# dongzhuoyao/self-guided-diffusion-models

Hardware: AMD Instinct MI355X
Metric: cfg_sampled_images_per_sec_64x64_1000step_ddpm (higher is better)
Workload: dtype f32 as 3xf16 split MFMA products, f32 accumulate; 1 GPU; IN64 unet_fast ch128 cluster-k5000 cond_scale=2 bs=40/GPU (UNet batch 80), 1000-step native DDPM; batch_per_gpu=40, unet_batch=80, precision_mode=f16x3, launch=hipGraph-captured step

## Files before the change

self-guided-diffusion-models_amd/csrc/attention.hip:

```cpp
#include "sgdm_common.h"
#include "../../include/sgdm_hip.h"

namespace {

constexpr int KT = 64;

template <int D>
__global__ __launch_bounds__(256) void attention_kernel(const float* __restrict__ q, int q_ld, int q_hs,
                                                        const float* __restrict__ k, const float* __restrict__ v,
                                                        int kv_ld, int kv_hs, int tq, int tk, float scale,
                                                        float* __restrict__ out, int out_ld,
                                                        float* __restrict__ lse,
                                                        const uint8_t* __restrict__ kmask = nullptr) {
    constexpr int LD = D + 4;
    constexpr int DT = (D + 31) / 32;
    constexpr int KT = D > 64 ? 32 : 64;
    __shared__ __attribute__((aligned(16))) float Ks[KT * LD];
    __shared__ __attribute__((aligned(16))) float Vs[KT * LD];

    const int tid = threadIdx.x, lane = tid & 63, wave = tid >> 6;
    const int li = lane & 31, lh = lane >> 5;
    const int head = blockIdx.y, b = blockIdx.z;
    const int qi = blockIdx.x * 128 + wave * 32 + li;
    const int qc = qi < tq ? qi : tq - 1;

    f32x4 qreg[D / 8];
    {
        const float* qp = q + ((long)b * tq + qc) * q_ld + head * q_hs;
#pragma unroll
        for (int s = 0; s < D / 8; ++s) {
            f32x4 t = *reinterpret_cast<const f32x4*>(qp + s * 8 + lh * 4);
            qreg[s] = t * scale;
        }
    }

    f32x16 oacc[DT];
#pragma unroll
    for (int i = 0; i < DT; ++i)
#pragma unroll
        for (int r = 0; r < 16; ++r) oacc[i][r] = 0.f;
    float m_run = -INFINITY, l_run = 0.f;

    const float* kb = k + (long)b * tk * kv_ld + head * kv_hs;
    const float* vb = v + (long)b * tk * kv_ld + head * kv_hs;

    for (int kt0 = 0; kt0 < tk; kt0 += KT) {
        __syncthreads();
        constexpr int VPR = D / 4;
        for (int idx = tid; idx < KT * VPR; idx += 256) {
            const int row = idx / VPR, c4 = idx % VPR;
            f32x4 kv4 = {0.f, 0.f, 0.f, 0.f}, vv4 = {0.f, 0.f, 0.f, 0.f};
            if (kt0 + row < tk) {
                kv4 = *reinterpret_cast<const f32x4*>(kb + (long)(kt0 + row) * kv_ld + c4 * 4);
                vv4 = *reinterpret_cast<const f32x4*>(vb + (long)(kt0 + row) * kv_ld + c4 * 4);
            }
            *reinterpret_cast<f32x4*>(Ks + row * LD + c4 * 4) = kv4;
            *reinterpret_cast<f32x4*>(Vs + row * LD + c4 * 4) = vv4;
        }
        __syncthreads();

#pragma unroll
        for (int st = 0; st < KT / 32; ++st) {
            if (kt0 + st * 32 >= tk) break;
            f32x16 sacc;
#pragma unroll
            for (int r = 0; r < 16; ++r) sacc[r] = 0.f;
#pragma unroll
            for (int s = 0; s < D / 8; ++s) {
                f32x4 kf = *reinterpret_cast<const f32x4*>(Ks + (st * 32 + li) * LD + s * 8 + lh * 4);
#pragma unroll
                for (int j = 0; j < 4; ++j) sacc = __builtin_amdgcn_mfma_f32_32x32x2f32(kf[j], qreg[s][j], sacc, 0, 0, 0);
            }
            unsigned dead = 0;
            if (kmask) {
#pragma unroll
                for (int r = 0; r < 16; ++r) {
                    const int key = kt0 + st * 32 + (r & 3) + 8 * (r >> 2) + 4 * lh;
                    const uint8_t keep = kmask[(long)b * tk + (key < tk ? key : tk - 1)];
                    dead |= (keep ? 0u : 1u) << r;
                }
            }
            float mx = -INFINITY;
#pragma unroll
            for (int r = 0; r < 16; ++r) {
                const int key = kt0 + st * 32 + (r & 3) + 8 * (r >> 2) + 4 * lh;
                const bool drop = key >= tk || ((dead >> r) & 1u);
                sacc[r] = drop ? -INFINITY : sacc[r];
                mx = fmaxf(mx, sacc[r]);
            }
            mx = fmaxf(mx, __shfl_xor(mx, 32, 64));
            const float m_new = fmaxf(m_run, mx);
            const float alpha = __expf(m_run - m_new);
            float psum = 0.f;
#pragma unroll
            for (int r = 0; r < 16; ++r) {
                sacc[r] = __expf(sacc[r] - m_new);
                psum += sacc[r];
            }
            l_run = l_run * alpha + psum;
            m_run = m_new;
#pragma unroll
            for (int dt = 0; dt < DT; ++dt) {
#pragma unroll
                for (int r = 0; r < 16; ++r) oacc[dt][r] *= alpha;
#pragma unroll
                for (int r = 0; r < 16; ++r) {
                    const int key = st * 32 + (r & 3) + 8 * (r >> 2) + 4 * lh;
                    float vf = 0.f;
                    if (D >= 32 || li < D) vf = Vs[key * LD + dt * 32 + li];
                    oacc[dt] = __builtin_amdgcn_mfma_f32_32x32x2f32(vf, sacc[r], oacc[dt], 0, 0, 0);
                }
            }
        }
    }
    const float l_tot = l_run + __shfl_xor(l_run, 32, 64);
    const float inv = 1.0f / l_tot;
    if (lse && qi < tq && lh == 0) lse[((long)b * gridDim.y + head) * tq + qi] = m_run + __logf(l_tot);
    if (qi < tq) {
        float* op = out + ((long)b * tq + qi) * out_ld + head * D;
#pragma unroll
        for (int dt = 0; dt < DT; ++dt)
#pragma unroll
            for (int r = 0; r < 16; ++r) {
                const int dd = dt * 32 + (r & 3) + 8 * (r >> 2) + 4 * lh;
                if (dd < D) op[dd] = oacc[dt][r] * inv;
            }
    }
}


__device__ __forceinline__ void split_f16(float v, _Float16& hi, _Float16& lo) {
    SGD_ROUNDED(v);
    hi = (_Float16)v;
    lo = (_Float16)(v - (float)hi);
}

template <int D>
__global__ __launch_bounds__(256) void attention_split_kernel(const float* __restrict__ q, int q_ld, int q_hs,
                                                              const float* __restrict__ k, const float* __restrict__ v,
                                                              int kv_ld, int kv_hs, int tq, int tk, float scale,
                                                              float* __restrict__ out, int out_ld,
                                                              float* __restrict__ lse) {
    constexpr int DT = (D + 31) / 32;
    constexpr int DP = DT * 32;
    constexpr int KS = (D + 15) / 16;
    constexpr int DK = KS * 16;
    constexpr int KT = D > 64 ? 32 : 64;
    constexpr int LDK = DK + 8;
    constexpr int LDV = KT + 8;
    __shared__ __attribute__((aligned(16))) _Float16 Kh[KT * LDK];
    __shared__ __attribute__((aligned(16))) _Float16 Kl[KT * LDK];
    __shared__ __attribute__((aligned(16))) _Float16 Vh[DP * LDV];
    __shared__ __attribute__((aligned(16))) _Float16 Vl[DP * LDV];

    const int tid = threadIdx.x, lane = tid & 63, wave = tid >> 6;
    const int li = lane & 31, lh = lane >> 5;
    const int head = blockIdx.y, b = blockIdx.z;
    const int qi = blockIdx.x * 128 + wave * 32 + li;
    const int qc = qi < tq ? qi : tq - 1;

    f16x8 qh[KS], ql[KS];
    {
        const float* qp = q + ((long)b * tq + qc) * q_ld + head * q_hs;
#pragma unroll
        for (int s = 0; s < KS; ++s)
#pragma unroll
            for (int j4 = 0; j4 < 2; ++j4) {
                const int c = s * 16 + lh * 8 + j4 * 4;
                f32x4 t = {0.f, 0.f, 0.f, 0.f};
                if (c < D) t = *reinterpret_cast<const f32x4*>(qp + c);
#pragma unroll
                for (int j = 0; j < 4; ++j) {
                    _Float16 h, l;
                    split_f16(t[j] * scale, h, l);
                    qh[s][j4 * 4 + j] = h;
                    ql[s][j4 * 4 + j] = l;
                }
            }
    }

    f32x16 oacc[DT];
#pragma unroll
    for (int i = 0; i < DT; ++i)
#pragma unroll
        for (int r = 0; r < 16; ++r) oacc[i][r] = 0.f;
    float m_run = -INFINITY, l_run = 0.f;
    constexpr float LOG2E = 1.4426950408889634f;
    constexpr float PSHIFT = 14.0f;

    const float* kb = k + (long)b * tk * kv_ld + head * kv_hs;
    const float* vb = v + (long)b * tk * kv_ld + head * kv_hs;

    if (DP > D) {
        for (int idx = tid; idx < (DP - D) * LDV; idx += 256) {
            Vh[D * LDV + idx] = (_Float16)0.f;
            Vl[D * LDV + idx] = (_Float16)0.f;
        }
    }

    constexpr int VPR = D / 4;
    constexpr int NKI = (KT * VPR + 255) / 256;
    constexpr int NVI = ((KT / 2) * VPR + 255) / 256;
    f32x4 kq[NKI], vq0[NVI], vq1[NVI];
    const int klast = tk - 1;
    auto request = [&](int kt0) __attribute__((always_inline)) {
#pragma unroll
        for (int i = 0; i < NKI; ++i) {
            int idx = tid + i * 256;
            idx = idx < KT * VPR ? idx : KT * VPR - 1;
            const int row = idx / VPR, c4 = idx % VPR;
            const int key = kt0 + row < tk ? kt0 + row : klast;
            kq[i] = *reinterpret_cast<const f32x4*>(kb + (long)key * kv_ld + c4 * 4);
        }
#pragma unroll
        for (int i = 0; i < NVI; ++i) {
            int idx = tid + i * 256;
            idx = idx < (KT / 2) * VPR ? idx : (KT / 2) * VPR - 1;
            const int key = kt0 + (idx / VPR) * 2, c4 = idx % VPR;
            vq0[i] = *reinterpret_cast<const f32x4*>(vb + (long)(key < tk ? key : klast) * kv_ld + c4 * 4);
            vq1[i] = *reinterpret_cast<const f32x4*>(vb + (long)(key + 1 < tk ? key + 1 : klast) * kv_ld + c4 * 4);
        }
    };
    request(0);
    for (int kt0 = 0; kt0 < tk; kt0 += KT) {
        __syncthreads();
#pragma unroll
        for (int i = 0; i < NKI; ++i) {
            const int idx = tid + i * 256;
            if (idx >= KT * VPR) break;
            const int row = idx / VPR, c4 = idx % VPR;
            f32x4 t = kq[i];
            if (kt0 + row >= tk) t = f32x4{0.f, 0.f, 0.f, 0.f};
            f16x4 h4, l4;
#pragma unroll
            for (int j = 0; j < 4; ++j) {
                _Float16 h, l;
                split_f16(t[j], h, l);
                h4[j] = h;
                l4[j] = l;
            }
            *reinterpret_cast<f16x4*>(Kh + row * LDK + c4 * 4) = h4;
            *reinterpret_cast<f16x4*>(Kl + row * LDK + c4 * 4) = l4;
        }
#pragma unroll
        for (int i = 0; i < NVI; ++i) {
            const int idx = tid + i * 256;
            if (idx >= (KT / 2) * VPR) break;
            const int kp = idx / VPR, c4 = idx % VPR;
            const int key = kp * 2;
            f32x4 t0 = vq0[i], t1 = vq1[i];
            if (kt0 + key >= tk) t0 = f32x4{0.f, 0.f, 0.f, 0.f};
            if (kt0 + key + 1 >= tk) t1 = f32x4{0.f, 0.f, 0.f, 0.f};
            const int kk = key & 15;
            const int pos = (key & ~15) + (((kk >> 2) & 1) << 3) + ((kk >> 3) << 2) + (kk & 3);
#pragma unroll
            for (int j = 0; j < 4; ++j) {
                _Float16 h0, l0, h1, l1;
                split_f16(t0[j], h0, l0);
                split_f16(t1[j], h1, l1);
                typedef _Float16 f16x2 __attribute__((ext_vector_type(2)));
                f16x2 hh = {h0, h1}, ll = {l0, l1};
                *reinterpret_cast<f16x2*>(Vh + (c4 * 4 + j) * LDV + pos) = hh;
                *reinterpret_cast<f16x2*>(Vl + (c4 * 4 + j) * LDV + pos) = ll;
            }
        }
        if (kt0 + KT < tk) request(kt0 + KT);
        __syncthreads();

#pragma unroll
        for (int st = 0; st < KT / 32; ++st) {
            if (kt0 + st * 32 >= tk) break;
            f32x16 sacc;
#pragma unroll
            for (int r = 0; r < 16; ++r) sacc[r] = 0.f;
#pragma unroll
            for (int s = 0; s < KS; ++s) {
                const f16x8 kh = *reinterpret_cast<const f16x8*>(Kh + (st * 32 + li) * LDK + s * 16 + lh * 8);
                const f16x8 kl = *reinterpret_cast<const f16x8*>(Kl + (st * 32 + li) * LDK + s * 16 + lh * 8);
                sacc = __builtin_amdgcn_mfma_f32_32x32x16_f16(kl, qh[s], sacc, 0, 0, 0);
                sacc = __builtin_amdgcn_mfma_f32_32x32x16_f16(kh, ql[s], sacc, 0, 0, 0);
                sacc = __builtin_amdgcn_mfma_f32_32x32x16_f16(kh, qh[s], sacc, 0, 0, 0);
            }
            float mx = -INFINITY;
#pragma unroll
            for (int r = 0; r < 16; ++r) {
                const int key = kt0 + st * 32 + (r & 3) + 8 * (r >> 2) + 4 * lh;
                if (key >= tk) sacc[r] = -INFINITY;
                mx = fmaxf(mx, sacc[r]);
            }
            mx = fmaxf(mx, __shfl_xor(mx, 32, 64));
            const float m_new = fmaxf(m_run, mx);
            const float alpha = __builtin_amdgcn_exp2f((m_run - m_new) * LOG2E);
            float psum = 0.f;
            const float mb = PSHIFT - m_new * LOG2E;
#pragma unroll
            for (int r = 0; r < 16; ++r) {
                sacc[r] = __builtin_amdgcn_exp2f(fmaf(sacc[r], LOG2E, mb));
                psum += sacc[r];
            }
            l_run = l_run * alpha + psum;
            m_run = m_new;
            f16x8 ph[2], pl[2];
#pragma unroll
            for (int s2 = 0; s2 < 2; ++s2)
#pragma unroll
                for (int j = 0; j < 8; ++j) {
                    _Float16 h, l;
                    split_f16(sacc[s2 * 8 + j], h, l);
                    ph[s2][j] = h;
                    pl[s2][j] = l;
                }
#pragma unroll
            for (int dt = 0; dt < DT; ++dt) {
#pragma unroll
                for (int r = 0; r < 16; ++r) oacc[dt][r] *= alpha;
#pragma unroll
                for (int s2 = 0; s2 < 2; ++s2) {
                    const f16x8 vh = *reinterpret_cast<const f16x8*>(Vh + (dt * 32 + li) * LDV + st * 32 + s2 * 16 + lh * 8);
                    const f16x8 vl = *reinterpret_cast<const f16x8*>(Vl + (dt * 32 + li) * LDV + st * 32 + s2 * 16 + lh * 8);
                    oacc[dt] = __builtin_amdgcn_mfma_f32_32x32x16_f16(vl, ph[s2], oacc[dt], 0, 0, 0);
                    oacc[dt] = __builtin_amdgcn_mfma_f32_32x32x16_f16(vh, pl[s2], oacc[dt], 0, 0, 0);
                    oacc[dt] = __builtin_amdgcn_mfma_f32_32x32x16_f16(vh, ph[s2], oacc[dt], 0, 0, 0);
                }
            }
        }
    }
    const float l_tot = l_run + __shfl_xor(l_run, 32, 64);
    const float inv = 1.0f / l_tot;
    if (lse && qi < tq && lh == 0) lse[((long)b * gridDim.y + head) * tq + qi] = m_run + __logf(l_tot) - PSHIFT * 0.6931471805599453f;
    if (qi < tq) {
        float* op = out + ((long)b * tq + qi) * out_ld + head * D;
#pragma unroll
        for (int dt = 0; dt < DT; ++dt)
#pragma unroll
            for (int g = 0; g < 4; ++g) {
                const int dd = dt * 32 + 8 * g + 4 * lh;
                if (dd >= D) continue;
                f32x4 o4;
#pragma unroll
                for (int j = 0; j < 4; ++j) o4[j] = oacc[dt][g * 4 + j] * inv;
                *reinterpret_cast<f32x4*>(op + dd) = o4;
            }
    }
}


template <int D>
__global__ __launch_bounds__(256) void attn_bwd_prep_kernel(const float* __restrict__ o, int o_ld,
                                                            const float* __restrict__ dout, int dout_ld, int heads,
                                                            int tq, float* __restrict__ dvec) {
    const long i = blockIdx.x * (long)blockDim.x + threadIdx.x;
    const long total = (long)gridDim.y * heads * tq;
    (void)total;
    const int b = blockIdx.y;
    if (i >= (long)heads * tq) return;
    const int head = i / tq, qi = i % tq;
    const float* op = o + ((long)b * tq + qi) * o_ld + head * D;
    const float* gp = dout + ((long)b * tq + qi) * dout_ld + head * D;
    float s = 0.f;
#pragma unroll
    for (int d4 = 0; d4 < D / 4; ++d4) {
        f32x4 a = *reinterpret_cast<const f32x4*>(op + d4 * 4), g = *reinterpret_cast<const f32x4*>(gp + d4 * 4);
        s += a[0] * g[0] + a[1] * g[1] + a[2] * g[2] + a[3] * g[3];
    }
    dvec[((long)b * heads + head) * tq + qi] = s;
}

template <int D, int SWEEP, bool MASKED = false>
__global__ __launch_bounds__(256) void attention_bwd_kernel(
    const float* __restrict__ q, int q_ld, int q_hs, const float* __restrict__ k, const float* __restrict__ v,
    int kv_ld, int kv_hs, const float* __restrict__ dout, int dout_ld, const float* __restrict__ lse,
    const float* __restrict__ dvec, int tq, int tk, float scale, float* __restrict__ dq, float* __restrict__ dk,
    float* __restrict__ dv, int heads, int mq, const uint8_t* __restrict__ kmask = nullptr) {
    constexpr int LD = D + 4;
    constexpr int DT = (D + 31) / 32;
    constexpr int TT = D > 64 ? 32 : 64;
    __shared__ __attribute__((aligned(16))) float Us[TT * LD];
    __shared__ __attribute__((aligned(16))) float Ws[TT * LD];
    __shared__ float Ls[TT], Ds[TT];
    __shared__ float Ms[MASKED ? TT : 1];

    const int tid = threadIdx.x, lane = tid & 63, wave = tid >> 6;
    const int li = lane & 31, lh = lane >> 5;
    const int b = blockIdx.z;
    const int head0 = mq ? 0 : blockIdx.y, head1 = mq ? heads : blockIdx.y + 1;
    const int own_n = SWEEP == 0 ? tk : tq;
    const int str_n = SWEEP == 0 ? tq : tk;
    const int oi = blockIdx.x * 128 + wave * 32 + li;
    const int oc = oi < own_n ? oi : own_n - 1;
    float own_keep = 1.f;
    if (MASKED && SWEEP == 0) own_keep = kmask[(long)b * tk + oc] ? 1.f : 0.f;

    f32x16 accA[DT], accB[DT];
#pragma unroll
    for (int i = 0; i < DT; ++i)
#pragma unroll
        for (int r = 0; r < 16; ++r) { accA[i][r] = 0.f; accB[i][r] = 0.f; }
    int head = head0;
    for (; head < head1; ++head) {
    const float* qb = q + (long)b * tq * q_ld + head * q_hs;
    const float* kb = k + (long)b * tk * kv_ld + head * kv_hs;
    const float* vb = v + (long)b * tk * kv_ld + head * kv_hs;
    const float* gb = dout + (long)b * tq * dout_ld + head * D;
    const float* lseb = lse + ((long)b * heads + head) * tq;
    const float* dvb = dvec + ((long)b * heads + head) * tq;

    f32x4 xf[D / 8], yf[D / 8];
    {
        const float* xp = SWEEP == 0 ? kb + (long)oc * kv_ld : qb + (long)oc * q_ld;
        const float* yp = SWEEP == 0 ? vb + (long)oc * kv_ld : gb + (long)oc * dout_ld;
#pragma unroll
        for (int s = 0; s < D / 8; ++s) {
            xf[s] = *reinterpret_cast<const f32x4*>(xp + s * 8 + lh * 4);
            yf[s] = *reinterpret_cast<const f32x4*>(yp + s * 8 + lh * 4);
        }
    }
    float own_lse = 0.f, own_d = 0.f;
    if (SWEEP == 1) { own_lse = lseb[oc]; own_d = dvb[oc]; }

    for (int t0 = 0; t0 < str_n; t0 += TT) {
        __syncthreads();
        constexpr int VPR = D / 4;
        constexpr int NI = (TT * VPR + 255) / 256;
        f32x4 ureg[NI], wreg[NI];
#pragma unroll
        for (int i = 0; i < NI; ++i) {
            int idx = tid + i * 256;
            idx = idx < TT * VPR ? idx : TT * VPR - 1;
            const int row = idx / VPR, c4 = idx % VPR;
            const long rr = t0 + row < str_n ? t0 + row : str_n - 1;
            if (SWEEP == 0) {
                ureg[i] = *reinterpret_cast<const f32x4*>(qb + rr * q_ld + c4 * 4);
                wreg[i] = *reinterpret_cast<const f32x4*>(gb + rr * dout_ld + c4 * 4);
            } else {
                ureg[i] = *reinterpret_cast<const f32x4*>(kb + rr * kv_ld + c4 * 4);
                wreg[i] = *reinterpret_cast<const f32x4*>(vb + rr * kv_ld + c4 * 4);
            }
        }
#pragma unroll
        for (int i = 0; i < NI; ++i) {
            const int idx = tid + i * 256;
            if (idx >= TT * VPR) break;
            const int row = idx / VPR, c4 = idx % VPR;
            f32x4 u = ureg[i], w = wreg[i];
            if (t0 + row >= str_n) { u = f32x4{0.f, 0.f, 0.f, 0.f}; w = u; }
            *reinterpret_cast<f32x4*>(Us + row * LD + c4 * 4) = u;
            *reinterpret_cast<f32x4*>(Ws + row * LD + c4 * 4) = w;
        }
        if (SWEEP == 0 && tid < TT) {
            const int r = t0 + tid;
            Ls[tid] = r < str_n ? lseb[r] : 0.f;
            Ds[tid] = r < str_n ? dvb[r] : 0.f;
        }
        if (MASKED && SWEEP == 1 && tid < TT) {
            const int r = t0 + tid;
            Ms[tid] = (r < str_n && kmask[(long)b * tk + r]) ? 1.f : 0.f;
        }
        __syncthreads();
#pragma unroll
        for (int st = 0; st < TT / 32; ++st) {
            if (t0 + st * 32 >= str_n) break;
            f32x16 sacc, pacc;
#pragma unroll
            for (int r = 0; r < 16; ++r) { sacc[r] = 0.f; pacc[r] = 0.f; }
#pragma unroll
            for (int s = 0; s < D / 8; ++s) {
                const f32x4 uf = *reinterpret_cast<const f32x4*>(Us + (st * 32 + li) * LD + s * 8 + lh * 4);
                const f32x4 wf = *reinterpret_cast<const f32x4*>(Ws + (st * 32 + li) * LD + s * 8 + lh * 4);
#pragma unroll
                for (int j = 0; j < 4; ++j) {
                    sacc = __builtin_amdgcn_mfma_f32_32x32x2f32(uf[j], xf[s][j], sacc, 0, 0, 0);
                    pacc = __builtin_amdgcn_mfma_f32_32x32x2f32(wf[j], yf[s][j], pacc, 0, 0, 0);
                }
            }
#pragma unroll
            for (int r = 0; r < 16; ++r) {
                const int srow = st * 32 + (r & 3) + 8 * (r >> 2) + 4 * lh;
                const bool ok = (t0 + srow < str_n) && (oi < own_n);
// ... 318 lines not shown
        float sum = 0.f;
        for (int c = 0; c < d; ++c) sum += __expf(qp[c] - m);
        const float inv = scale / sum;
        float* op = out + ((long)b * tq + i) * out_ld + head * q_hs;
        for (int e = 0; e < d; ++e) {
            float acc = 0.f;
            for (int c = 0; c < d; ++c) acc += __expf(qp[c] - m) * inv * ctx[c * (d + 1) + e];
            op[e] = acc;
        }
    }
}

__global__ __launch_bounds__(256) void linear_attention_bwd_kernel(const float* __restrict__ q, int q_ld, int q_hs,
                                                                   const float* __restrict__ k, const float* __restrict__ v,
                                                                   int kv_ld, int kv_hs, int tq, int tk, int d, float scale,
                                                                   const uint8_t* __restrict__ kmask,
                                                                   const float* __restrict__ dout, int dout_ld,
                                                                   float* __restrict__ dq, float* __restrict__ dk,
                                                                   float* __restrict__ dv, int tr) {
    extern __shared__ float sh[];
    const int P = d + 1;
    float* ctx = sh;
    float* dctx = ctx + d * P;
    float* cmax = dctx + d * P;
    float* csum = cmax + d;
    float* colt = csum + d;
    float* S = colt + d;
    float* G = S + tr * d;
    float* T = G + tr * d;
    float* rmax = T + tr * d;
    float* rinv = rmax + tr;
    float* rdot = rinv + tr;
    const int head = blockIdx.x, b = blockIdx.y, tid = threadIdx.x;
    const float* kb = k + (long)b * tk * kv_ld + head * kv_hs;
    const float* vb = v + (long)b * tk * kv_ld + head * kv_hs;
    const uint8_t* mb = kmask ? kmask + (long)b * tk : nullptr;
    for (int c = tid; c < d; c += 256) {
        float m = -INFINITY;
        for (int j = 0; j < tk; ++j) m = fmaxf(m, (mb && !mb[j]) ? -3.402823466e38f : kb[(long)j * kv_ld + c]);
        float sum = 0.f;
        for (int j = 0; j < tk; ++j) sum += __expf(((mb && !mb[j]) ? -3.402823466e38f : kb[(long)j * kv_ld + c]) - m);
        cmax[c] = m;
        csum[c] = sum;
    }
    __syncthreads();
    for (int i = tid; i < d * d; i += 256) {
        const int c = i / d, e = i % d;
        float acc = 0.f;
        for (int j = 0; j < tk; ++j) {
            const bool ok = !mb || mb[j];
            const float kk = ok ? kb[(long)j * kv_ld + c] : -3.402823466e38f;
            const float vv = ok ? vb[(long)j * kv_ld + e] : 0.f;
            acc += __expf(kk - cmax[c]) / csum[c] * vv;
        }
        ctx[c * P + e] = acc;
        dctx[c * P + e] = 0.f;
    }
    __syncthreads();
    for (int i0 = 0; i0 < tq; i0 += tr) {
        const int rows = tq - i0 < tr ? tq - i0 : tr;
        if (tid < rows) {
            const float* qp = q + ((long)b * tq + i0 + tid) * q_ld + head * q_hs;
            float m = -INFINITY;
            for (int c = 0; c < d; ++c) m = fmaxf(m, qp[c]);
            float sum = 0.f;
            for (int c = 0; c < d; ++c) sum += __expf(qp[c] - m);
            rmax[tid] = m;
            rinv[tid] = 1.f / sum;
        }
        __syncthreads();
        for (int idx = tid; idx < rows * d; idx += 256) {
            const int r = idx / d, c = idx % d;
            const long row = (long)b * tq + i0 + r;
            S[idx] = __expf(q[row * q_ld + head * q_hs + c] - rmax[r]) * rinv[r];
            G[idx] = dout[row * dout_ld + head * q_hs + c];
        }
        __syncthreads();
        for (int i = tid; i < d * d; i += 256) {
            const int c = i / d, e = i % d;
            float acc = 0.f;
            for (int r = 0; r < rows; ++r) acc += S[r * d + c] * G[r * d + e];
            dctx[c * P + e] += scale * acc;
        }
        for (int idx = tid; idx < rows * d; idx += 256) {
            const int r = idx / d, c = idx % d;
            float acc = 0.f;
            for (int e = 0; e < d; ++e) acc += G[r * d + e] * ctx[c * P + e];
            T[idx] = scale * acc;
        }
        __syncthreads();
        if (tid < rows) {
            float acc = 0.f;
            for (int c = 0; c < d; ++c) acc += S[tid * d + c] * T[tid * d + c];
            rdot[tid] = acc;
        }
        __syncthreads();
        for (int idx = tid; idx < rows * d; idx += 256) {
            const int r = idx / d, c = idx % d;
            dq[((long)b * tq + i0 + r) * q_ld + head * q_hs + c] = S[idx] * (T[idx] - rdot[r]);
        }
        __syncthreads();
    }
    for (int c = tid; c < d; c += 256) {
        float acc = 0.f;
        for (int e = 0; e < d; ++e) acc += dctx[c * P + e] * ctx[c * P + e];
        colt[c] = acc;
    }
    __syncthreads();
    for (int idx = tid; idx < tk * d; idx += 256) {
        const int j = idx / d, c = idx % d;
        const bool ok = !mb || mb[j];
        float gk = 0.f, gv = 0.f;
        if (ok) {
            const float kt = __expf(kb[(long)j * kv_ld + c] - cmax[c]) / csum[c];
            float acc = 0.f;
            for (int e = 0; e < d; ++e) acc += dctx[c * P + e] * vb[(long)j * kv_ld + e];
            gk = kt * (acc - colt[c]);
            for (int c2 = 0; c2 < d; ++c2) gv += __expf(kb[(long)j * kv_ld + c2] - cmax[c2]) / csum[c2] * dctx[c2 * P + c];
        }
        dk[((long)b * tk + j) * kv_ld + head * kv_hs + c] = gk;
        dv[((long)b * tk + j) * kv_ld + head * kv_hs + c] = gv;
    }
}


}

extern "C" int sgd_attention(const float* q, int32_t q_ld, int32_t q_hs, const float* k, const float* v,
                             int32_t kv_ld, int32_t kv_hs, int32_t batch, int32_t heads, int32_t tq, int32_t tk,
                             int32_t d, float scale, float* out, int32_t out_ld, float* lse, void* stream) {
    SGD_CLEAR_ERR();
    if (!q || !k || !v || !out || batch <= 0 || heads <= 0 || tq <= 0 || tk <= 0) return SGD_ERR_ARG;
    if ((q_ld & 3) || (q_hs & 3) || (kv_ld & 3) || (kv_hs & 3)) return SGD_ERR_ARG;
    if ((((uintptr_t)q) | ((uintptr_t)k) | ((uintptr_t)v)) & 15) return SGD_ERR_ARG;
    dim3 grid((tq + 127) / 128, heads, batch);
    hipStream_t st = (hipStream_t)stream;
    switch (d) {
        case 16: hipLaunchKernelGGL((attention_kernel<16>), grid, dim3(256), 0, st, q, q_ld, q_hs, k, v, kv_ld, kv_hs, tq, tk, scale, out, out_ld, lse); break;
        case 32: hipLaunchKernelGGL((attention_kernel<32>), grid, dim3(256), 0, st, q, q_ld, q_hs, k, v, kv_ld, kv_hs, tq, tk, scale, out, out_ld, lse); break;
        case 64: hipLaunchKernelGGL((attention_kernel<64>), grid, dim3(256), 0, st, q, q_ld, q_hs, k, v, kv_ld, kv_hs, tq, tk, scale, out, out_ld, lse); break;
        case 128: hipLaunchKernelGGL((attention_kernel<128>), grid, dim3(256), 0, st, q, q_ld, q_hs, k, v, kv_ld, kv_hs, tq, tk, scale, out, out_ld, lse); break;
        default: return SGD_ERR_ARG;
    }
    return sgd_check_launch();
}

extern "C" int sgd_attention_split(const float* q, int32_t q_ld, int32_t q_hs, const float* k, const float* v,
                                   int32_t kv_ld, int32_t kv_hs, int32_t batch, int32_t heads, int32_t tq, int32_t tk,
                                   int32_t d, float scale, float* out, int32_t out_ld, float* lse, void* stream) {
    SGD_CLEAR_ERR();
    if (!q || !k || !v || !out || batch <= 0 || heads <= 0 || tq <= 0 || tk <= 0) return SGD_ERR_ARG;
    if ((q_ld & 3) || (q_hs & 3) || (kv_ld & 3) || (kv_hs & 3) || (out_ld & 3)) return SGD_ERR_ARG;
    if ((((uintptr_t)q) | ((uintptr_t)k) | ((uintptr_t)v) | ((uintptr_t)out)) & 15) return SGD_ERR_ARG;
    dim3 grid((tq + 127) / 128, heads, batch);
    hipStream_t st = (hipStream_t)stream;
    switch (d) {
        case 16: hipLaunchKernelGGL((attention_split_kernel<16>), grid, dim3(256), 0, st, q, q_ld, q_hs, k, v, kv_ld, kv_hs, tq, tk, scale, out, out_ld, lse); break;
        case 32: hipLaunchKernelGGL((attention_split_kernel<32>), grid, dim3(256), 0, st, q, q_ld, q_hs, k, v, kv_ld, kv_hs, tq, tk, scale, out, out_ld, lse); break;
        case 64: hipLaunchKernelGGL((attention_split_kernel<64>), grid, dim3(256), 0, st, q, q_ld, q_hs, k, v, kv_ld, kv_hs, tq, tk, scale, out, out_ld, lse); break;
        case 128: hipLaunchKernelGGL((attention_split_kernel<128>), grid, dim3(256), 0, st, q, q_ld, q_hs, k, v, kv_ld, kv_hs, tq, tk, scale, out, out_ld, lse); break;
        default: return SGD_ERR_ARG;
    }
    return sgd_check_launch();
}

extern "C" int sgd_attention_bwd(const float* q, int32_t q_ld, int32_t q_hs, const float* k, const float* v,
                                 int32_t kv_ld, int32_t kv_hs, const float* o, int32_t o_ld, const float* dout,
                                 int32_t dout_ld, const float* lse, float* dvec, int32_t batch, int32_t heads,
                                 int32_t tq, int32_t tk, int32_t d, float scale, float* dq, float* dk, float* dv,
                                 void* stream) {
    SGD_CLEAR_ERR();
    if (!q || !k || !v || !o || !dout || !lse || !dvec || !dq || !dk || !dv || batch <= 0 || heads <= 0 || tq <= 0 ||
        tk <= 0)
        return SGD_ERR_ARG;
    if ((q_ld & 3) || (q_hs & 3) || (kv_ld & 3) || (kv_hs & 3) || (o_ld & 3) || (dout_ld & 3)) return SGD_ERR_ARG;
    hipStream_t st = (hipStream_t)stream;
    const int mq = (kv_hs == 0 && heads > 1) ? 1 : 0;
    dim3 gp((heads * tq + 255) / 256, batch), gkv((tk + 127) / 128, mq ? 1 : heads, batch), gq((tq + 127) / 128, heads, batch);
#define SGD_ATTN_BWD(DD)                                                                                              \
    hipLaunchKernelGGL((attn_bwd_prep_kernel<DD>), gp, dim3(256), 0, st, o, o_ld, dout, dout_ld, heads, tq, dvec);      \
    hipLaunchKernelGGL((attention_bwd_kernel<DD, 0>), gkv, dim3(256), 0, st, q, q_ld, q_hs, k, v, kv_ld, kv_hs, dout,   \
                       dout_ld, lse, dvec, tq, tk, scale, dq, dk, dv, heads, mq);                                      \
    hipLaunchKernelGGL((attention_bwd_kernel<DD, 1>), gq, dim3(256), 0, st, q, q_ld, q_hs, k, v, kv_ld, kv_hs, dout,    \
                       dout_ld, lse, dvec, tq, tk, scale, dq, dk, dv, heads, 0);
    switch (d) {
        case 16: SGD_ATTN_BWD(16) break;
        case 32: SGD_ATTN_BWD(32) break;
        case 64: SGD_ATTN_BWD(64) break;
        case 128: SGD_ATTN_BWD(128) break;
        default: return SGD_ERR_ARG;
    }
#undef SGD_ATTN_BWD
    return sgd_check_launch();
}

extern "C" int sgd_attention_bwd_split(const float* q, int32_t q_ld, int32_t q_hs, const float* k, const float* v,
                                       int32_t kv_ld, int32_t kv_hs, const float* o, int32_t o_ld, const float* dout,
                                       int32_t dout_ld, const float* lse, float* dvec, int32_t batch, int32_t heads,
                                       int32_t tq, int32_t tk, int32_t d, float scale, float* dq, float* dk, float* dv,
                                       void* stream) {
    SGD_CLEAR_ERR();
    if (!q || !k || !v || !o || !dout || !lse || !dvec || !dq || !dk || !dv || batch <= 0 || heads <= 0 || tq <= 0 ||
        tk <= 0)
        return SGD_ERR_ARG;
    if ((q_ld & 3) || (q_hs & 3) || (kv_ld & 3) || (kv_hs & 3) || (o_ld & 3) || (dout_ld & 3)) return SGD_ERR_ARG;
    hipStream_t st = (hipStream_t)stream;
    const int mq = (kv_hs == 0 && heads > 1) ? 1 : 0;
    dim3 gp((heads * tq + 255) / 256, batch), gkv((tk + 127) / 128, mq ? 1 : heads, batch), gq((tq + 127) / 128, heads, batch);
#define SGD_ATTN_BWD_S(DD)                                                                                            \
    hipLaunchKernelGGL((attn_bwd_prep_kernel<DD>), gp, dim3(256), 0, st, o, o_ld, dout, dout_ld, heads, tq, dvec);      \
    hipLaunchKernelGGL((attention_bwd_split_kernel<DD, 0>), gkv, dim3(256), 0, st, q, q_ld, q_hs, k, v, kv_ld, kv_hs,   \
                       dout, dout_ld, lse, dvec, tq, tk, scale, dq, dk, dv, heads, mq);                                \
    hipLaunchKernelGGL((attention_bwd_split_kernel<DD, 1>), gq, dim3(256), 0, st, q, q_ld, q_hs, k, v, kv_ld, kv_hs,    \
                       dout, dout_ld, lse, dvec, tq, tk, scale, dq, dk, dv, heads, 0);
    switch (d) {
        case 16: SGD_ATTN_BWD_S(16) break;
        case 32: SGD_ATTN_BWD_S(32) break;
        case 64: SGD_ATTN_BWD_S(64) break;
        default: return SGD_ERR_ARG;
    }
#undef SGD_ATTN_BWD_S
    return sgd_check_launch();
}

extern "C" int sgd_attention_masked(const float* q, int32_t q_ld, int32_t q_hs, const float* k, const float* v,
                                    int32_t kv_ld, int32_t kv_hs, const uint8_t* kmask, int32_t batch, int32_t heads,
                                    int32_t tq, int32_t tk, int32_t d, float scale, float* out, int32_t out_ld, float* lse,
                                    void* stream) {
    SGD_CLEAR_ERR();
    if (!q || !k || !v || !out || batch <= 0 || heads <= 0 || tq <= 0 || tk <= 0) return SGD_ERR_ARG;
    if ((q_ld & 3) || (q_hs & 3) || (kv_ld & 3) || (kv_hs & 3)) return SGD_ERR_ARG;
    if ((((uintptr_t)q) | ((uintptr_t)k) | ((uintptr_t)v)) & 15) return SGD_ERR_ARG;
    dim3 grid((tq + 127) / 128, heads, batch);
    hipStream_t st = (hipStream_t)stream;
    switch (d) {
        case 16: hipLaunchKernelGGL((attention_kernel<16>), grid, dim3(256), 0, st, q, q_ld, q_hs, k, v, kv_ld, kv_hs, tq, tk, scale, out, out_ld, lse, kmask); break;
        case 32: hipLaunchKernelGGL((attention_kernel<32>), grid, dim3(256), 0, st, q, q_ld, q_hs, k, v, kv_ld, kv_hs, tq, tk, scale, out, out_ld, lse, kmask); break;
        case 64: hipLaunchKernelGGL((attention_kernel<64>), grid, dim3(256), 0, st, q, q_ld, q_hs, k, v, kv_ld, kv_hs, tq, tk, scale, out, out_ld, lse, kmask); break;
        case 128: hipLaunchKernelGGL((attention_kernel<128>), grid, dim3(256), 0, st, q, q_ld, q_hs, k, v, kv_ld, kv_hs, tq, tk, scale, out, out_ld, lse, kmask); break;
        default: return SGD_ERR_ARG;
    }
    return sgd_check_launch();
}

extern "C" int sgd_linear_attention(const float* q, int32_t q_ld, int32_t q_hs, const float* k, const float* v,
                                    int32_t kv_ld, int32_t kv_hs, const uint8_t* kmask, int32_t batch, int32_t heads,
                                    int32_t tq, int32_t tk, int32_t d, float scale, float* out, int32_t out_ld,
                                    void* stream) {
    SGD_CLEAR_ERR();
    if (!q || !k || !v || !out || batch <= 0 || heads <= 0 || tq <= 0 || tk <= 0 || d <= 0 || d > 128) return SGD_ERR_ARG;
    const size_t smem = ((size_t)d * (d + 1) + 2 * d) * sizeof(float);
    static bool attr = false;
    if (!attr) {
        (void)hipFuncSetAttribute((const void*)linear_attention_kernel, hipFuncAttributeMaxDynamicSharedMemorySize, 80 * 1024);
        attr = true;
    }
    hipLaunchKernelGGL(linear_attention_kernel, dim3(heads, batch), dim3(256), smem, (hipStream_t)stream, q, q_ld, q_hs, k,
                       v, kv_ld, kv_hs, tq, tk, d, scale, kmask, out, out_ld);
    return sgd_check_launch();
}

extern "C" int sgd_attention_masked_bwd(const float* q, int32_t q_ld, int32_t q_hs, const float* k, const float* v,
                                        int32_t kv_ld, int32_t kv_hs, const uint8_t* kmask, const float* o, int32_t o_ld,
                                        const float* dout, int32_t dout_ld, const float* lse, float* dvec, int32_t batch,
                                        int32_t heads, int32_t tq, int32_t tk, int32_t d, float scale, float* dq, float* dk,
                                        float* dv, void* stream) {
    SGD_CLEAR_ERR();
    if (!q || !k || !v || !kmask || !o || !dout || !lse || !dvec || !dq || !dk || !dv || batch <= 0 || heads <= 0 || tq <= 0 ||
        tk <= 0)
        return SGD_ERR_ARG;
    if ((q_ld & 3) || (q_hs & 3) || (kv_ld & 3) || (kv_hs & 3) || (o_ld & 3) || (dout_ld & 3)) return SGD_ERR_ARG;
    if (kv_hs == 0 && heads > 1) return SGD_ERR_ARG;
    hipStream_t st = (hipStream_t)stream;
    dim3 gp((heads * tq + 255) / 256, batch), gkv((tk + 127) / 128, heads, batch), gq((tq + 127) / 128, heads, batch);
#define SGD_ATTN_BWD_M(DD)                                                                                            \
    hipLaunchKernelGGL((attn_bwd_prep_kernel<DD>), gp, dim3(256), 0, st, o, o_ld, dout, dout_ld, heads, tq, dvec);      \
    hipLaunchKernelGGL((attention_bwd_kernel<DD, 0, true>), gkv, dim3(256), 0, st, q, q_ld, q_hs, k, v, kv_ld, kv_hs,   \
                       dout, dout_ld, lse, dvec, tq, tk, scale, dq, dk, dv, heads, 0, kmask);                          \
    hipLaunchKernelGGL((attention_bwd_kernel<DD, 1, true>), gq, dim3(256), 0, st, q, q_ld, q_hs, k, v, kv_ld, kv_hs,    \
                       dout, dout_ld, lse, dvec, tq, tk, scale, dq, dk, dv, heads, 0, kmask);
    switch (d) {
        case 16: SGD_ATTN_BWD_M(16) break;
        case 32: SGD_ATTN_BWD_M(32) break;
        case 64: SGD_ATTN_BWD_M(64) break;
        case 128: SGD_ATTN_BWD_M(128) break;
        default: return SGD_ERR_ARG;
    }
#undef SGD_ATTN_BWD_M
    return sgd_check_launch();
}

extern "C" int sgd_linear_attention_bwd(const float* q, int32_t q_ld, int32_t q_hs, const float* k, const float* v,
                                        int32_t kv_ld, int32_t kv_hs, const uint8_t* kmask, const float* dout,
                                        int32_t dout_ld, int32_t batch, int32_t heads, int32_t tq, int32_t tk, int32_t d,
                                        float scale, float* dq, float* dk, float* dv, void* stream) {
    SGD_CLEAR_ERR();
    if (!q || !k || !v || !dout || !dq || !dk || !dv || batch <= 0 || heads <= 0 || tq <= 0 || tk <= 0 || d <= 0 || d > 128)
        return SGD_ERR_ARG;
    const int tr = d > 64 ? 8 : 32;
    const size_t smem = ((size_t)2 * d * (d + 1) + 3 * d + (size_t)3 * tr * d + 3 * tr) * sizeof(float);
    static bool attr = false;
    if (!attr) {
        (void)hipFuncSetAttribute((const void*)linear_attention_bwd_kernel, hipFuncAttributeMaxDynamicSharedMemorySize,
                                  152 * 1024);
        attr = true;
    }
    hipLaunchKernelGGL(linear_attention_bwd_kernel, dim3(heads, batch), dim3(256), smem, (hipStream_t)stream, q, q_ld, q_hs,
                       k, v, kv_ld, kv_hs, tq, tk, d, scale, kmask, dout, dout_ld, dq, dk, dv, tr);
    return sgd_check_launch();
}
```

Before: 2.526 images/s.

## Widen split-f16 attention blocks to 8 waves and vectorize f16 splitting

```diff
diff --git a/self-guided-diffusion-models_amd/csrc/attention.hip b/self-guided-diffusion-models_amd/csrc/attention.hip
--- a/self-guided-diffusion-models_amd/csrc/attention.hip
+++ b/self-guided-diffusion-models_amd/csrc/attention.hip
@@ -1,4 +1,6 @@
+#include <type_traits>
 #include "sgdm_common.h"
+#include "prologue.h"
 #include "../../include/sgdm_hip.h"
 
 namespace {
@@ -135,12 +137,26 @@
     lo = (_Float16)(v - (float)hi);
 }
 
-template <int D>
-__global__ __launch_bounds__(256) void attention_split_kernel(const float* __restrict__ q, int q_ld, int q_hs,
-                                                              const float* __restrict__ k, const float* __restrict__ v,
-                                                              int kv_ld, int kv_hs, int tq, int tk, float scale,
-                                                              float* __restrict__ out, int out_ld,
-                                                              float* __restrict__ lse) {
+__device__ __forceinline__ void split4_f16_after_exp(f32x4 v, u32x2& h, u32x2& l) {
+    float a = v[0], b = v[1], c = v[2], d = v[3];
+#if defined(__HIP_DEVICE_COMPILE__)
+    asm("s_nop 0" : "+v"(a), "+v"(b), "+v"(c), "+v"(d));
+#endif
+    split4_f16(f32x4{a, b, c, d}, h, l);
+}
+
+__device__ __forceinline__ f16x8 frag8(u32x2 a, u32x2 b) {
+    return __builtin_bit_cast(f16x8, u32x4_t{a.x, a.y, b.x, b.y});
+}
+
+template <int D, int NW>
+__global__ __launch_bounds__(NW * 64, (NW == 4 && D <= 64) ? 2 : 1)
+void attention_split_kernel(const float* __restrict__ q, int q_ld, int q_hs,
+                                                                  const float* __restrict__ k, const float* __restrict__ v,
+                                                                  int kv_ld, int kv_hs, int tq, int tk, float scale,
+                                                                  float* __restrict__ out, int out_ld,
+                                                                  float* __restrict__ lse) {
+    constexpr int NT = NW * 64;
     constexpr int DT = (D + 31) / 32;
     constexpr int DP = DT * 32;
     constexpr int KS = (D + 15) / 16;
@@ -156,27 +172,25 @@
     const int tid = threadIdx.x, lane = tid & 63, wave = tid >> 6;
     const int li = lane & 31, lh = lane >> 5;
     const int head = blockIdx.y, b = blockIdx.z;
-    const int qi = blockIdx.x * 128 + wave * 32 + li;
+    const int qi = blockIdx.x * (NW * 32) + wave * 32 + li;
     const int qc = qi < tq ? qi : tq - 1;
 
     f16x8 qh[KS], ql[KS];
     {
         const float* qp = q + ((long)b * tq + qc) * q_ld + head * q_hs;
 #pragma unroll
-        for (int s = 0; s < KS; ++s)
+        for (int s = 0; s < KS; ++s) {
+            u32x2 h[2], l[2];
 #pragma unroll
             for (int j4 = 0; j4 < 2; ++j4) {
                 const int c = s * 16 + lh * 8 + j4 * 4;
                 f32x4 t = {0.f, 0.f, 0.f, 0.f};
                 if (c < D) t = *reinterpret_cast<const f32x4*>(qp + c);
-#pragma unroll
-                for (int j = 0; j < 4; ++j) {
-                    _Float16 h, l;
-                    split_f16(t[j] * scale, h, l);
-                    qh[s][j4 * 4 + j] = h;
-                    ql[s][j4 * 4 + j] = l;
-                }
-            }
+                split4_f16(t * scale, h[j4], l[j4]);
+            }
+            qh[s] = frag8(h[0], h[1]);
+            ql[s] = frag8(l[0], l[1]);
+        }
     }
 
     f32x16 oacc[DT];
@@ -192,21 +206,21 @@
     const float* vb = v + (long)b * tk * kv_ld + head * kv_hs;
 
     if (DP > D) {
-        for (int idx = tid; idx < (DP - D) * LDV; idx += 256) {
+        for (int idx = tid; idx < (DP - D) * LDV; idx += NT) {
             Vh[D * LDV + idx] = (_Float16)0.f;
             Vl[D * LDV + idx] = (_Float16)0.f;
         }
     }
 
     constexpr int VPR = D / 4;
-    constexpr int NKI = (KT * VPR + 255) / 256;
-    constexpr int NVI = ((KT / 2) * VPR + 255) / 256;
+    constexpr int NKI = (KT * VPR + NT - 1) / NT;
+    constexpr int NVI = ((KT / 2) * VPR + NT - 1) / NT;
     f32x4 kq[NKI], vq0[NVI], vq1[NVI];
     const int klast = tk - 1;
     auto request = [&](int kt0) __attribute__((always_inline)) {
 #pragma unroll
         for (int i = 0; i < NKI; ++i) {
-            int idx = tid + i * 256;
+            int idx = tid + i * NT;
             idx = idx < KT * VPR ? idx : KT * VPR - 1;
             const int row = idx / VPR, c4 = idx % VPR;
             const int key = kt0 + row < tk ? kt0 + row : klast;
@@ -214,37 +228,29 @@
         }
 #pragma unroll
         for (int i = 0; i < NVI; ++i) {
-            int idx = tid + i * 256;
+            int idx = tid + i * NT;
             idx = idx < (KT / 2) * VPR ? idx : (KT / 2) * VPR - 1;
             const int key = kt0 + (idx / VPR) * 2, c4 = idx % VPR;
             vq0[i] = *reinterpret_cast<const f32x4*>(vb + (long)(key < tk ? key : klast) * kv_ld + c4 * 4);
             vq1[i] = *reinterpret_cast<const f32x4*>(vb + (long)(key + 1 < tk ? key + 1 : klast) * kv_ld + c4 * 4);
         }
     };
-    request(0);
-    for (int kt0 = 0; kt0 < tk; kt0 += KT) {
-        __syncthreads();
+    auto stage = [&](int kt0) __attribute__((always_inline)) {
 #pragma unroll
         for (int i = 0; i < NKI; ++i) {
-            const int idx = tid + i * 256;
+            const int idx = tid + i * NT;
             if (idx >= KT * VPR) break;
             const int row = idx / VPR, c4 = idx % VPR;
             f32x4 t = kq[i];
             if (kt0 + row >= tk) t = f32x4{0.f, 0.f, 0.f, 0.f};
-            f16x4 h4, l4;
-#pragma unroll
-            for (int j = 0; j < 4; ++j) {
-                _Float16 h, l;
-                split_f16(t[j], h, l);
-                h4[j] = h;
-                l4[j] = l;
-            }
-            *reinterpret_cast<f16x4*>(Kh + row * LDK + c4 * 4) = h4;
-            *reinterpret_cast<f16x4*>(Kl + row * LDK + c4 * 4) = l4;
+            u32x2 h4, l4;
+            split4_f16(t, h4, l4);
+            *reinterpret_cast<u32x2*>(Kh + row * LDK + c4 * 4) = h4;
+            *reinterpret_cast<u32x2*>(Kl + row * LDK + c4 * 4) = l4;
         }
 #pragma unroll
         for (int i = 0; i < NVI; ++i) {
-            const int idx = tid + i * 256;
+            const int idx = tid + i * NT;
             if (idx >= (KT / 2) * VPR) break;
             const int kp = idx / VPR, c4 = idx % VPR;
             const int key = kp * 2;
@@ -254,19 +260,18 @@
             const int kk = key & 15;
             const int pos = (key & ~15) + (((kk >> 2) & 1) << 3) + ((kk >> 3) << 2) + (kk & 3);
 #pragma unroll
-            for (int j = 0; j < 4; ++j) {
-                _Float16 h0, l0, h1, l1;
-                split_f16(t0[j], h0, l0);
-                split_f16(t1[j], h1, l1);
-                typedef _Float16 f16x2 __attribute__((ext_vector_type(2)));
-                f16x2 hh = {h0, h1}, ll = {l0, l1};
-                *reinterpret_cast<f16x2*>(Vh + (c4 * 4 + j) * LDV + pos) = hh;
-                *reinterpret_cast<f16x2*>(Vl + (c4 * 4 + j) * LDV + pos) = ll;
-            }
-        }
-        if (kt0 + KT < tk) request(kt0 + KT);
-        __syncthreads();
-
+            for (int j2 = 0; j2 < 2; ++j2) {
+                u32x2 hh, ll;
+                split4_f16(f32x4{t0[2 * j2], t1[2 * j2], t0[2 * j2 + 1], t1[2 * j2 + 1]}, hh, ll);
+                *reinterpret_cast<uint32_t*>(Vh + (c4 * 4 + 2 * j2) * LDV + pos) = hh.x;
+                *reinterpret_cast<uint32_t*>(Vl + (c4 * 4 + 2 * j2) * LDV + pos) = ll.x;
+                *reinterpret_cast<uint32_t*>(Vh + (c4 * 4 + 2 * j2 + 1) * LDV + pos) = hh.y;
+                *reinterpret_cast<uint32_t*>(Vl + (c4 * 4 + 2 * j2 + 1) * LDV + pos) = ll.y;
+            }
+        }
+    };
+    auto tile = [&](auto partial, int kt0) __attribute__((always_inline)) {
+        constexpr bool PARTIAL = decltype(partial)::value;
 #pragma unroll
         for (int st = 0; st < KT / 32; ++st) {
             if (kt0 + st * 32 >= tk) break;
@@ -284,8 +289,10 @@
             float mx = -INFINITY;
 #pragma unroll
             for (int r = 0; r < 16; ++r) {
-                const int key = kt0 + st * 32 + (r & 3) + 8 * (r >> 2) + 4 * lh;
-                if (key >= tk) sacc[r] = -INFINITY;
+                if (PARTIAL) {
+                    const int key = kt0 + st * 32 + (r & 3) + 8 * (r >> 2) + 4 * lh;
+                    if (key >= tk) sacc[r] = -INFINITY;
+                }
                 mx = fmaxf(mx, sacc[r]);
             }
             mx = fmaxf(mx, __shfl_xor(mx, 32, 64));
@@ -302,14 +309,16 @@
             m_run = m_new;
             f16x8 ph[2], pl[2];
 #pragma unroll
-            for (int s2 = 0; s2 < 2; ++s2)
-#pragma unroll
-                for (int j = 0; j < 8; ++j) {
-                    _Float16 h, l;
-                    split_f16(sacc[s2 * 8 + j], h, l);
-                    ph[s2][j] = h;
-                    pl[s2][j] = l;
-                }
+            for (int s2 = 0; s2 < 2; ++s2) {
+                u32x2 h[2], l[2];
+#pragma unroll
+                for (int j4 = 0; j4 < 2; ++j4) {
+                    const int r0 = s2 * 8 + j4 * 4;
+                    split4_f16_after_exp(f32x4{sacc[r0], sacc[r0 + 1], sacc[r0 + 2], sacc[r0 + 3]}, h[j4], l[j4]);
+                }
+                ph[s2] = frag8(h[0], h[1]);
+                pl[s2] = frag8(l[0], l[1]);
+            }
 #pragma unroll
             for (int dt = 0; dt < DT; ++dt) {
 #pragma unroll
@@ -324,6 +333,15 @@
                 }
             }
         }
+    };
+    request(0);
+    for (int kt0 = 0; kt0 < tk; kt0 += KT) {
+        __syncthreads();
+        stage(kt0);
+        if (kt0 + KT < tk) request(kt0 + KT);
+        __syncthreads();
+        if (kt0 + KT > tk) tile(std::true_type{}, kt0);
+        else tile(std::false_type{}, kt0);
     }
     const float l_tot = l_run + __shfl_xor(l_run, 32, 64);
     const float inv = 1.0f / l_tot;
@@ -948,15 +966,25 @@
     if (!q || !k || !v || !out || batch <= 0 || heads <= 0 || tq <= 0 || tk <= 0) return SGD_ERR_ARG;
     if ((q_ld & 3) || (q_hs & 3) || (kv_ld & 3) || (kv_hs & 3) || (out_ld & 3)) return SGD_ERR_ARG;
     if ((((uintptr_t)q) | ((uintptr_t)k) | ((uintptr_t)v) | ((uintptr_t)out)) & 15) return SGD_ERR_ARG;
-    dim3 grid((tq + 127) / 128, heads, batch);
+    const bool wide = tq > 128 && d <= 64;
+    dim3 grid4((tq + 127) / 128, heads, batch), grid8((tq + 255) / 256, heads, batch);
     hipStream_t st = (hipStream_t)stream;
+#define SGD_ATTN_SPLIT(DD)                                                                                                          \
+    if (wide)                                                                                                                       \
+        hipLaunchKernelGGL((attention_split_kernel<DD, 8>), grid8, dim3(512), 0, st, q, q_ld, q_hs, k, v, kv_ld, kv_hs, tq, tk, scale,  \
+                           out, out_ld, lse);                                                                                       \
+    else                                                                                                                            \
+        hipLaunchKernelGGL((attention_split_kernel<DD, 4>), grid4, dim3(256), 0, st, q, q_ld, q_hs, k, v, kv_ld, kv_hs, tq, tk, scale,  \
+                           out, out_ld, lse);                                                                                       \
+    break
     switch (d) {
-        case 16: hipLaunchKernelGGL((attention_split_kernel<16>), grid, dim3(256), 0, st, q, q_ld, q_hs, k, v, kv_ld, kv_hs, tq, tk, scale, out, out_ld, lse); break;
-        case 32: hipLaunchKernelGGL((attention_split_kernel<32>), grid, dim3(256), 0, st, q, q_ld, q_hs, k, v, kv_ld, kv_hs, tq, tk, scale, out, out_ld, lse); break;
-        case 64: hipLaunchKernelGGL((attention_split_kernel<64>), grid, dim3(256), 0, st, q, q_ld, q_hs, k, v, kv_ld, kv_hs, tq, tk, scale, out, out_ld, lse); break;
-        case 128: hipLaunchKernelGGL((attention_split_kernel<128>), grid, dim3(256), 0, st, q, q_ld, q_hs, k, v, kv_ld, kv_hs, tq, tk, scale, out, out_ld, lse); break;
+        case 16: SGD_ATTN_SPLIT(16);
+        case 32: SGD_ATTN_SPLIT(32);
+        case 64: SGD_ATTN_SPLIT(64);
+        case 128: hipLaunchKernelGGL((attention_split_kernel<128, 4>), grid4, dim3(256), 0, st, q, q_ld, q_hs, k, v, kv_ld, kv_hs, tq, tk, scale, out, out_ld, lse); break;
         default: return SGD_ERR_ARG;
     }
+#undef SGD_ATTN_SPLIT
     return sgd_check_launch();
 }
 
```

After: 2.530 images/s, median of 2. About the same (+0.2%).
